# tudocomp/tudocomp

Measured on AMD Instinct MI355X. Metric: input MB/s end-to-end lcpcomp+huffman, higher is better.
Workload: dtype u32

## Files before the change

### tudocomp_amd/csrc/api_compress.hip

```cpp
#include "api.hpp"
#include "bitsink.hpp"

#include <vector>

using namespace tdc;

namespace tdc {

void validate_device_text(Ctx& c, const u8* d_text, size_t n) {
    if (!(c.hist_ptr == d_text && c.hist_n == n)) {
        const size_t mark = c.arena.mark();
        u32* d_hist = c.arena.get<u32>(256);
        HIP_TRY(hipMemsetAsync(d_hist, 0, 256 * sizeof(u32), c.stream));
        text_histogram_add(c, d_text, n, d_hist);
        text_histogram_finish(c, d_text, n, d_hist);
        c.arena.release(mark);
    }
    u8 last = 1;
    HIP_TRY(hipMemcpyAsync(&last, d_text + n - 1, 1, hipMemcpyDeviceToHost, c.stream));
    HIP_TRY(hipStreamSynchronize(c.stream));
    const u32 zeros = c.hist_cache[0];
    if (last != 0) throw ArgError{TDC_GPU_ERR_NO_SENTINEL, "text does not end with a 0 sentinel"};
    if (zeros != 1) throw ArgError{TDC_GPU_ERR_ARG, "text contains 0 bytes besides the sentinel (escape the input first)"};
}

static bool early_is_planned(const Ctx& c, size_t n, u32 threshold, int flatten, int strategy, int enc_coder, const u8* d_text) {
    return strategy == TDC_GPU_COMP_ARRAYS && flatten && enc_coder == 0 && d_text && c.enc_early && c.enc_rec && c.huff_ok &&
           n >= (c.enc_early >= 2 ? (size_t)1 : ((size_t)1 << 20)) && threshold >= 2;
}

void run_textds(Ctx& c, const u8* d_text, size_t n, DevArrays& A, tdc_gpu_stats* st, Events* ev, bool want_phi, const CandWant* cw) {
    A.sa = c.arena.get<u32>(n);
    A.isa = c.arena.get<u32>(n);
    A.phi = nullptr;
    A.plcp = c.arena.get<u32>(n);
    u32* d_max = c.arena.get<u32>(1);
    SAStats ss;
    SAExtra ex;
    ex.lcp8 = c.arena.get<u8>(n + 64);
    const int e0 = ev ? ev->tick() : 0;
    build_suffix_array(c, d_text, n, A.sa, A.isa, &ss, &ex);
    const int e1 = ev ? ev->tick() : 0;
    int e2;
    if (!(ex.mode == 1 && !want_phi && c.phi_lazy)) A.phi = c.arena.get<u32>(n);
    if (ex.mode == 1) {
        CandFused* cf = nullptr;
        if (cw && c.fused_cand && !A.phi && fused_scatter_has_image(c, n)) {
            cf = &A.cand;
            cf->threshold = cw->threshold;
            cf->lcut = factorize_arrays_lcut0(c, n, cw->threshold);
            cf->cls = c.arena.get<u8>(n);
            if (cf->lcut) cf->res8 = c.arena.get<u8>(n);
            if (cw->flen8) cf->flen8 = A.fs.flen8 = c.arena.get<u8>(n + 64); else cf->flen = A.fs.flen = c.arena.get<u32>(n);
            if (c.sel_tile_counts) cf->tilecnt = c.arena.get<u32>(cdiv(n, SEL_TILE_CLASSES));
            cf->acc = c.arena.get<u32>((size_t)CF_COPIES * CF_ACC);
            cf->lvlhist = c.arena.get<u32>(128);
            cf->entries = cf->lvlhist + 64;
        }
        build_isa_phi_plcp_fused(c, A.sa, ex.lcp8, n, A.isa, A.phi, A.plcp, d_max, cf);
        e2 = ev ? ev->tick() : 0;
    } else {
        build_phi(c, A.sa, n, A.phi);
        e2 = ev ? ev->tick() : 0;
        build_plcp(c, d_text, n, A.phi, A.plcp, d_max);
    }
    const int e3 = ev ? ev->tick() : 0;
    A.maxlcp = c.read(d_max);
    if (st) {
        st->maxlcp = A.maxlcp;
        sa_stats(st, ss, &ex);
        if (ev) { ev->span(&st->ms_sa, e0, e1); ev->span(&st->ms_phi, e1, e2); ev->span(&st->ms_plcp, e2, e3); }
    }
}

constexpr size_t FLAT_CHUNK_MIN = (size_t)16 << 20;
constexpr size_t FLAT_CHUNK_MAX = 8;

void run_factorize(Ctx& c, size_t n, DevArrays& A, u32 threshold, int flatten, tdc_gpu_stats* st, Events* ev, int strategy,
                   int enc_coder, const u8* d_text) {
    if (!A.fs.flen) A.fs.flen = c.arena.get<u32>(n);
    A.fs.owner = c.arena.get<u32>(n);
    A.fs.fsrc = c.arena.get<u32>(n);
    A.fs.fpos = c.arena.get<u32>(n);
    A.fs.flenl = threshold >= 2 ? A.fs.fpos + (n + 1) / 2 : nullptr;
    A.fs.cls = c.arena.get<u8>(n + 64);
    const bool early_planned = early_is_planned(c, n, threshold, flatten, strategy, enc_coder, d_text);
    if (early_planned && c.flen_bytes && !A.fs.flen8) A.fs.flen8 = c.arena.get<u8>(n + 64);
    A.fs.want_owner_rem = early_planned ? (u32)c.owner_rem : 0u;
    FactorizeStats fz;
    FlattenStats fl;
    const int e0 = ev ? ev->tick() : 0;
    if (strategy == TDC_GPU_COMP_PLCPPEAKS) plcp_peaks_factorize(c, n, A.phi, A.plcp, threshold, A.fs, &fz.factors);
    else if (strategy == TDC_GPU_COMP_MAXLCP) factorize_max_lcp(c, n, A.isa, A.phi, A.plcp, A.maxlcp, threshold, A.fs, &fz);
    else if (strategy == TDC_GPU_COMP_HEAP) factorize_max_heap(c, n, A.sa, A.isa, A.plcp, A.maxlcp, threshold, A.fs, &fz);
    else factorize_arrays(c, n, A.sa, A.isa, A.phi, A.plcp, A.maxlcp, threshold, A.fs, &fz, A.cand.filled ? &A.cand : nullptr);
    const int e1 = ev ? ev->tick() : 0;
    const bool early = flatten && enc_coder == 0 && d_text && c.enc_early && c.huff_ok && n >= (c.enc_early >= 2 ? (size_t)1 : ((size_t)1 << 20)) &&
                       A.fs.have_list && A.fs.have_cls && A.fs.flenl && A.fs.nfact > 0;
    if (!early) expand_flen8(c, n, A.fs);
    if (early) {
        A.early = encode_early_reserve(c, n, c.enc_rec ? A.fs.nfact : 0);
        u32 K = c.flatten_chunks ? (u32)c.flatten_chunks : (u32)std::min<size_t>(A.fs.nfact / FLAT_CHUNK_MIN, FLAT_CHUNK_MAX);
        K = flatten_chunk_count(K, A.fs.nfact);
        const bool packed = K >= 2 && encode_early_chunks(c, n, A.fs, A.early, K, align_up(encode_bound_coder(n, enc_coder) + 16, 8));
        if (!packed && c.flatten_chunks < 2) K = 1;
        c.wait_for(c.copy_stream, c.stream);
        flatten_factors(c, n, A.fs, &fl, [&](int round) {
            StreamSwap sw(c, c.copy_stream);
            if (round == 1 || round == 2) encode_early_run(c, d_text, n, A.fs, enc_coder, A.early, false);
            else if (round == 0) encode_early_run(c, d_text, n, A.fs, enc_coder, A.early, true);
        }, c.enc_rec ? encode_early_rec(A.early) : nullptr, K,
        packed ? std::function<void(u32, size_t)>([&](u32 k, size_t) { encode_early_chunk_done(c, d_text, n, A.fs, A.early, k); }) : std::function<void(u32, size_t)>());
    } else if (flatten) {
        flatten_factors(c, n, A.fs, &fl);
    } else {
        materialize_sources(c, n, A.fs);
    }
    const int e2 = ev ? ev->tick() : 0;
    if (st) {
        st->factors = fz.factors; st->entries = fz.entries; st->pushes = fz.pushes;
        st->levels = fz.levels; st->mis_rounds = fz.rounds; st->small_levels = fz.small_levels; st->purges = fz.purges; st->window_pass = fz.window_pass; st->window_lcut = fz.window_lcut; st->eager_levels = fz.eager_levels; st->eager_phases = fz.eager_phases;
        st->probes = fz.probes; st->max_push_targets = fz.max_push_targets;
        st->num_flattened = fl.num_flattened; st->max_depth_lb = fl.max_depth_lb; st->flatten_rounds = fl.rounds;
        st->ranges_early = A.early ? encode_early_packed(A.early) : 0u;
        if (ev) { ev->span(&st->ms_factorize, e0, e1); ev->span(&st->ms_flatten, e1, e2); }
    }
}

u8* TextUpload::send(const uint8_t* text, size_t n) {
    if (n < ((size_t)1 << 26)) return upload_plain(c, text, n);
    u8* d_text = c.arena.get<u8>(n + 64);
    u32* d_hist = c.arena.get<u32>(256);
    HIP_TRY(hipMemsetAsync(d_hist, 0, 256 * sizeof(u32), c.stream));
    c.wait_for(c.copy_stream, c.stream);
    const bool try_pre = c.wsort_overlap && c.wpre && wsort_applicable(c, n);
    const size_t CH = try_pre ? (size_t)c.upload_chunks : 8;
    std::vector<size_t> coff;
    {
        std::vector<double> w(CH, 1.0);
        if (try_pre) {
            const size_t T = std::min<size_t>((size_t)c.upload_tail_n, CH - 1);
            double f = 1.0;
            for (size_t k = 0; k < T; ++k) { f *= (double)c.upload_tail_pct / 100.0; w[CH - T + k] = f; }
        }
        double tot = 0; for (double x : w) tot += x;
        coff.push_back(0);
        double acc = 0;
        for (size_t k = 0; k + 1 < CH; ++k) {
            acc += w[k];
            size_t o = ((size_t)((double)n * (acc / tot)) + 4095) & ~(size_t)4095;
            if (o <= coff.back()) o = coff.back() + 4096;
            if (o >= n) break;
            coff.push_back(o);
        }
        coff.push_back(n);
    }
    const size_t nch = coff.size() - 1;
    if (nch > Ctx::CHUNK_EVENTS) throw HipError{hipErrorUnknown, "upload: more chunks than chunk events", (int)__LINE__};
    size_t queued = 0;
    auto queue_copies = [&](size_t upto) {
        for (; queued < nch && queued < upto; ++queued) {
            const size_t off = coff[queued] + (queued ? 64 : 0), end = std::min(coff[queued + 1] + 64, n);
            if (end > off) HIP_TRY(hipMemcpyAsync(d_text + off, text + off, end - off, hipMemcpyHostToDevice, c.copy_stream));
            HIP_TRY(hipEventRecord(c.ev_chunk[queued], c.copy_stream));
// ... 666 lines not shown
```

### tudocomp_amd/csrc/api_ctx.hip

```cpp
#include "api.hpp"
#include "huffman_host.hpp"

#include <strings.h>
#include <ctype.h>

using namespace tdc;

namespace tdc {

int lcpcomp_enc_coder(int coder) {
    const int base = coder & 0xFF, k = coder >> 8;
    if (base == TDC_GPU_CODER_SLE) {
        if (k < 0 || k > 7) throw ArgError{TDC_GPU_ERR_ARG, "sle: kmer must be in 1..7"};
        return 3 | ((k ? k : 3) << 8);
    }
    if (k == 0 && base == TDC_GPU_CODER_HUFF) return 0;
    if (k == 0 && base == TDC_GPU_CODER_ARITH) return 1;
    if (k == 0 && base == TDC_GPU_CODER_ASCII) return 2;
    throw ArgError{TDC_GPU_ERR_UNSUPPORTED, "lcpcomp: coder must be huff, arithmetic, ascii or sle"};
}

void reserve_arena(Ctx& c, size_t bytes) {
    if (c.arena.size < bytes) {
        size_t fr = 0, tot = 0;
// ... 56 lines not shown
    { "phi_lazy",         [](Ctx& c, long v) { c.phi_lazy = v != 0; } },
    { "fs_pair",          [](Ctx& c, long v) { c.fs_pair = v != 0; } },
    { "enc_early",        [](Ctx& c, long v) { c.enc_early = (int)v; } },
    { "owner_rem",        [](Ctx& c, long v) { c.owner_rem = (int)std::min<long>(std::max<long>(v, 0), 8); } },
    { "enc_rec",          [](Ctx& c, long v) { c.enc_rec = v != 0; } },
    { "level_purge",      [](Ctx& c, long v) { c.level_purge = v != 0; } },
    { "level_log",        [](Ctx& c, long v) { c.level_log = v != 0; } },
    { "eager",            [](Ctx& c, long v) { c.eager_levels = v != 0; } },
    { "eager_dump",       [](Ctx& c, long v) { c.eager_dump = v != 0; } },
    { "flen_bytes",       [](Ctx& c, long v) { c.flen_bytes = v != 0; } },
    { "flatten_steps",    [](Ctx& c, long v) { c.flatten_steps = v <= 0 ? (1 << 30) : clampi(v, 1, 1 << 30); } },
    { "flatten_growth",   [](Ctx& c, long v) { c.flatten_growth = clampi(v, 2, 1 << 20); } },
    { "sa_refine",        [](Ctx& c, long v) { c.sa_refine = v != 0; } },
    { "sa_pairs",         [](Ctx& c, long v) { c.sa_pairs = v != 0; } },
    { "sa_stars",         [](Ctx& c, long v) { c.sa_stars = v != 0; } },
    { "sa_fused_init",    [](Ctx& c, long v) { c.sa_fused_init = v != 0; } },
    { "sa_init_syms",     [](Ctx& c, long v) { c.sa_init_syms = clampi(v, 0, 64); } },
    { "radix_lds",        [](Ctx& c, long v) { c.radix_lds = (v >= 0 && v <= 2) ? (int)v : 2; } },
    { "xcd_remap",        [](Ctx& c, long v) { c.xcd_remap = (v >= 0 && v <= 2) ? (int)v : 0; } },
    { "bucket_scatter",   [](Ctx& c, long v) { c.bucket_scatter = v ? 1 : 0; } },
    { "ssort",            [](Ctx& c, long v) { c.ssort = v ? 1 : 0; } },
    { "ssort_levels",     [](Ctx& c, long v) { c.ssort_levels = (v >= 1 && v <= 3) ? (int)v : 0; } },
    { "msd_partition",    [](Ctx& c, long v) { c.msd_partition = v ? 1 : 0; } },
    { "wsort",            [](Ctx& c, long v) { c.wsort = v ? 1 : 0; } },
    { "wsort_min",        [](Ctx& c, long v) { c.wsort_min = v < 4096 ? 4096 : (size_t)v; } },
    { "wsort_syms",       [](Ctx& c, long v) { c.wsort_syms = (v >= 4 && v <= 64) ? (int)v : 0; } },
    { "wsort_kw",         [](Ctx& c, long v) { c.wsort_kw = (v == 1 || v == 2) ? (int)v : 0; } },
    { "wsort_rounds",     [](Ctx& c, long v) { c.wsort_rounds = clampi(v, 0, 100); } },
    { "wsort_smallrun",   [](Ctx& c, long v) { c.wsort_small = v ? 1 : 0; } },
    { "wsort_overlap",    [](Ctx& c, long v) { c.wsort_overlap = v ? 1 : 0; } },
    { "wsort_predig",     [](Ctx& c, long v) { c.wsort_predig = v ? 1 : 0; } },
    { "wsort_prehist",    [](Ctx& c, long v) { c.wsort_prehist = v ? 1 : 0; } },
    { "sa_seg_bigcap",    [](Ctx& c, long v) { c.sa_seg_bigcap = clampi(v, 0, 65536); } },
    { "sa_seg_rounds",    [](Ctx& c, long v) { c.sa_seg_rounds = clampi(v, 0, 2); } },
    { "wsort_run_streams",[](Ctx& c, long v) { c.wsort_run_streams = v != 0; } },
    { "wsort_predig_skip",[](Ctx& c, long v) { c.wsort_predig_skip = clampi(v, 0, 24); } },
    { "wsort_fuse",       [](Ctx& c, long v) { c.wsort_fuse = v ? 1 : 0; } },
    { "wsort_order",      [](Ctx& c, long v) { c.wsort_order = v ? 1 : 0; } },
    { "wsort_two",        [](Ctx& c, long v) { c.wsort_two = (v >= 0 && v <= 2) ? (int)v : 0; } },
    { "wsort_leaf",       [](Ctx& c, long v) { c.wsort_leaf = v == 1024 ? 1024 : 2048; } },
    { "wsort_pack",       [](Ctx& c, long v) { c.wsort_pack = (v == 1024 || v == 4096) ? (int)v : 2048; } },
    { "wsort_cmax",       [](Ctx& c, long v) { c.wsort_cmax = clampi(v, 8, 64); } },
    { "wsort_log",        [](Ctx& c, long v) { c.wsort_log = v != 0; } },
    { "upload_chunks",    [](Ctx& c, long v) { c.upload_chunks = clampi(v, 4, 24); } },
    { "upload_tail_n",    [](Ctx& c, long v) { c.upload_tail_n = clampi(v, 0, 12); } },
    { "upload_tail_pct",  [](Ctx& c, long v) { c.upload_tail_pct = clampi(v, 30, 100); } },
    { "arena_log",        [](Ctx& c, long v) { c.arena_log = v != 0; } },
};
constexpr size_t NOPTIONS = sizeof(OPTIONS) / sizeof(OPTIONS[0]);
const OptionDef FOLD_OPTIONS[] = {
    { "fused_cand",       [](Ctx& c, long v) { c.fused_cand = v != 0; } },
    { "sel_tile_counts",  [](Ctx& c, long v) { c.sel_tile_counts = v != 0; } },
    { "flatten_chunks",   [](Ctx& c, long v) { c.flatten_chunks = clampi(v, 0, (long)FLATTEN_MAX_CHUNKS); } },
    { "repair_recount",   [](Ctx& c, long v) { c.repair_recount = v != 0; } },
    { "repair_table_bits",[](Ctx& c, long v) { c.repair_table_bits = v == 0 ? 0 : clampi(v, 8, 30); } },
    { "repair_log",       [](Ctx& c, long v) { c.repair_log = v != 0; } },
    { "repair_dec_rounds",[](Ctx& c, long v) { c.repair_dec_rounds = clampi(v, 1, 1 << 24); } },
    { "lz_batch_hash_bits",[](Ctx& c, long v) { c.lz_batch_hash_bits = clampi(v, 0, 24); } },
};
constexpr size_t NFOLD = sizeof(FOLD_OPTIONS) / sizeof(FOLD_OPTIONS[0]);
const OptionDef* find_option(const char* name) {
    if (!name) return nullptr;
    if (!strncasecmp(name, "TDC_GPU_", 8)) name += 8;
    for (size_t i = 0; i < NOPTIONS; ++i) if (!strcasecmp(name, OPTIONS[i].name)) return &OPTIONS[i];
    for (size_t i = 0; i < NFOLD; ++i) if (!strcasecmp(name, FOLD_OPTIONS[i].name)) return &FOLD_OPTIONS[i];
    return nullptr;
}
void apply_env_options(tdc_gpu_ctx* ctx) {
    const char* on = getenv("TDC_GPU_DEBUG_KNOBS");
    if (!on || atoi(on) == 0) return;
    for (size_t i = 0; i < NOPTIONS + NFOLD; ++i) {
        const OptionDef& o = i < NOPTIONS ? OPTIONS[i] : FOLD_OPTIONS[i - NOPTIONS];
        char var[64] = "TDC_GPU_";
        size_t k = 8;
        for (const char* q = o.name; *q && k + 1 < sizeof(var); ++q) var[k++] = (char)toupper((unsigned char)*q);
        var[k] = 0;
        if (const char* m = getenv(var)) o.set(ctx->c, atol(m));
    }
}
}

int tdc_gpu_ctx_set_option(tdc_gpu_ctx* ctx, const char* name, long value) {
    if (!ctx) return TDC_GPU_ERR_ARG;
    const OptionDef* o = find_option(name);
    if (!o) return TDC_GPU_ERR_ARG;
    o->set(ctx->c, value);
    return TDC_GPU_OK;
}
int tdc_gpu_option_count(void) { return (int)NOPTIONS; }
const char* tdc_gpu_option_name(int i) { return (i >= 0 && (size_t)i < NOPTIONS) ? OPTIONS[i].name : nullptr; }

int tdc_gpu_ctx_create(int device, tdc_gpu_ctx** out) {
    if (!out) return TDC_GPU_ERR_ARG;
    *out = nullptr;
    int count = 0;
    if (hipGetDeviceCount(&count) != hipSuccess || count <= 0) { (void)hipGetLastError(); return TDC_GPU_ERR_HIP; }
    if (device < 0 || device >= count) return TDC_GPU_ERR_ARG;
    tdc_gpu_ctx* ctx = new (std::nothrow) tdc_gpu_ctx();
    if (!ctx) return TDC_GPU_ERR_OOM;
    ctx->c.huff_ok = huffman_selfcheck();
    ctx->c.device = device;
    ctx->c.wpre = &ctx->pre;
    DeviceGuard dg(device);
    try {
        HIP_TRY(dg.enter());
        HIP_TRY(hipStreamCreateWithFlags(&ctx->c.stream, hipStreamNonBlocking));
// ... 171 lines not shown
```

### tudocomp_amd/csrc/common.hpp

```cpp
#pragma once

#include <hip/hip_runtime.h>
#include <stdint.h>
#include <stddef.h>
#include <stdio.h>
#include <string.h>

namespace tdc {

typedef uint8_t  u8;
typedef uint32_t u32;
typedef uint16_t u16;
typedef uint64_t u64;

constexpr u32 NONE32 = 0xFFFFFFFFu;
constexpr int WAVE = 64;

enum {
    TDC_OK = 0,
    TDC_ERR_HIP = -1,
    TDC_ERR_ARG = -2,
    TDC_ERR_NO_SENTINEL = -3,
    TDC_ERR_TOO_LARGE = -4,
    TDC_ERR_OOM = -5,
// ... 111 lines not shown
    int level_purge = 1;
    int enc_rec = 1;
    int owner_rem = 8;
    int enc_early = 1;
    int fused_cand = 1;
    int sel_tile_counts = 1;
    int fs_pair = 1;
    int small_big = 1;
    int small_pipeline = 1;
    int sa_pairs = 1;
    int sa_stars = 1;
    int sa_refine = 1;
    int sa_fused_init = 1;
    int radix_lds = 1;
    int xcd_remap = 1;
    int window_src = 1;
    int window_lcut = 56;
    int window_halo = 320;
    size_t dec_seg = 0;
    bool phi_lazy = true;
    int dec_lean = 1;
    int dec_parse = 1;
    int window_force_fail = 0;
    int window_large_lists = 0;
    int ssort = 1;
    int ssort_levels = 0;
    int wsort = 1;
    size_t wsort_min = (size_t)1 << 20;
    int wsort_syms = 0;
    int wsort_kw = 0;
    int wsort_rounds = 24;
    int wsort_cmax = 24;
    int wsort_overlap = 1;
    int wsort_prehist = 1;
    bool wsort_count_nonheads = true;
    int sa_seg_bigcap = 65536;
    int sa_seg_rounds = 2;
    int wsort_run_streams = 1;
    int wsort_predig_skip = 4;
    int wsort_predig = 1;
    int wsort_two = 0;
    int wsort_leaf = 2048;
    int wsort_pack = 1024;
    int wsort_order = 1;
    int wsort_fuse = 1;
    int wsort_small = 0;
    int msd_partition = 1;
    int bucket_scatter = 1;
    int upload_tail_n = 3, upload_tail_pct = 60;
    int upload_chunks = 16;
    int flatten_steps = 1;
    int flatten_growth = 8;
    int flatten_chunks = 0;
    int sa_init_syms = 0;
    int dec_done = 1;
    int repair_recount = 0;
    int repair_table_bits = 0;
    int repair_log = 0;
    int repair_dec_rounds = 1024;
    int lz_batch_hash_bits = 0;
    int dec_log = 0, bwt_log = 0, pipe_log = 0, level_log = 0, wsort_log = 0, eager_dump = 0, small_prof = 0, arena_log = 0;

    u32 hist_cache[256] = {};
    const u8* hist_ptr = nullptr;
    size_t hist_n = 0;
    hipStream_t copy_stream = nullptr;
    hipStream_t aux_stream = nullptr;
    hipEvent_t ev_join = nullptr;
    static constexpr size_t CHUNK_EVENTS = 32;
    hipEvent_t ev_chunk[CHUNK_EVENTS] = {};
    hipEvent_t ev_dig2 = nullptr;
    struct WPre* wpre = nullptr;
    u8* d2h_host = nullptr;
    size_t d2h_cap = 0;
    size_t d2h_done = 0;

    bool profiling = false;
    KernelProfile kprof[K_CLASS_COUNT];
    struct Pending { hipEvent_t a, b; int cls; u64 bytes; };
    Pending* pend = nullptr;
    int npend = 0, pend_cap = 0;
    hipEvent_t* ev_pool = nullptr;
    int ev_pool_size = 0, ev_pool_used = 0;

    int prof_begin(int cls, u64 bytes) {
        if (!profiling || npend >= pend_cap || ev_pool_used + 2 > ev_pool_size) return -1;
        Pending& p = pend[npend];
        p.a = ev_pool[ev_pool_used++]; p.b = ev_pool[ev_pool_used++]; p.cls = cls; p.bytes = bytes;
        HIP_TRY(hipEventRecord(p.a, stream));
        return npend++;
    }
    void prof_end(int idx) { if (idx >= 0) HIP_TRY(hipEventRecord(pend[idx].b, stream)); }
    void wait_for(hipStream_t waiter, hipStream_t signaller) {
        HIP_TRY(hipEventRecord(ev_join, signaller));
        HIP_TRY(hipStreamWaitEvent(waiter, ev_join, 0));
    }
    struct ProfScope {
        Ctx& c; int idx;
        ProfScope(Ctx& ctx, int cls, u64 bytes) : c(ctx), idx(ctx.prof_begin(cls, bytes)) {}
        ~ProfScope() { if (idx >= 0) (void)hipEventRecord(c.pend[idx].b, c.stream); }
    };
    void prof_collect() {
        for (int i = 0; i < npend; ++i) {
            float t = 0;
            HIP_TRY(hipEventElapsedTime(&t, pend[i].a, pend[i].b));
            KernelProfile& k = kprof[pend[i].cls];
// ... 274 lines not shown
```

### tudocomp_amd/csrc/encode.hip

```cpp
#include "stages.hpp"
#include "bytestages.hpp"
#include "bitsink.hpp"
#include "prim.hpp"
#include "huffman_host.hpp"
#include "arith.hpp"
#include "decode.hpp"

#include <string.h>
#include <algorithm>
#include <vector>

namespace tdc {

struct CodeTable {
    u64 code[256];
    u8 len[256];
};

struct EncParams {
    u32 W, lbits, dbits, flen_min;
    u32 raw_literals;
    u32 ascii;
    u32 uni;
};
// ... 309 lines not shown
            }
        }
    }
    u64 total;
    const u64 ex = block_exclusive_sum<u64, 4>((u64)sum | ((u64)starts << 40), sm, total);
    const u64 excl = ex & ((1ull << 40) - 1ull);
    if (p0 >= n) return;
    u32 k = REC ? tile_rank[tile] + (u32)(ex >> 40) : 0u;
    BitSink sink;
    sink.out = out;
    sink.pos = base_bits + tile_off[tile] + excl;
    sink.acc = 0;
    sink.cnt = 0;
    u32 prev = prev0;
#pragma unroll
    for (int j = 0; j < ENC_PER_THREAD; ++j) {
        const size_t p = p0 + j;
        if (p < n) {
            const u32 o = cl[j];
            if (o == 0u) {
                if (p == 0 || prev != 0u) {
                    const u32 run = REC ? ((k < z ? rec[k].x : (u32)n) - (u32)p) : fl[j];
                    sink.append(1, 1); sink.append(run, P.dbits);
                }
                if (A.litidx) {
                    const u32 q = A.litidx[p];
                    if (A.amark[q]) sink.append(A.fval[q], 64);
                    if (q == A.lc_index) { sink.append(A.pp_lb, 64); sink.append(~0ull, 64); }
                }
                else if (P.raw_literals) sink.append(ch[j], 8);
                else sink.append(code[ch[j]], clen[ch[j]]);
            } else if (o == 2u) {
                if (p == 0 || prev != 0u) sink.append(0, 1);
                if (REC) {
                    const uint4 r = rec[k++];
                    sink.append(r.w, P.W);
                    sink.append(r.y - P.flen_min, P.lbits);
                } else {
                    sink.append(fsrc[p], P.W);
                    sink.append(fl[j] - P.flen_min, P.lbits);
                }
            }
            prev = o;
        }
    }
    sink.flush();
}

struct PackBounds { u32 end[16]; };
__global__ void pick_u64_kernel(const u64* __restrict__ excl, PackBounds b, u32 parts, u64* __restrict__ out) {
    const u32 q = threadIdx.x;
    if (q < parts) out[q] = (q + 1 < parts) ? excl[b.end[q]] : 0ull;
}
__global__ void range_tiles_kernel(const u32* __restrict__ fpos, u32 z, u32 K, u32* __restrict__ out) {
    const u32 k = threadIdx.x;
    if (k + 1 < K) out[k] = fpos[(u32)((u64)z * (k + 1) / K)] / (u32)ENC_TILE;
}

size_t encode_bound(size_t n) { return 12 * n + 4096; }
size_t encode_bound_coder(size_t n, int coder) { return ((coder & 0xFF) == 2 ? 24 : 12) * n + ((coder & 0xFF) == 3 ? 32768 : 4096); }
size_t encode_bound_uni(size_t n, int coder) { return (coder == 4 ? 8 : coder == 5 ? 9 : 6) * n + 64; }

size_t encode_huff(Ctx& c, const u8* text, size_t n, FactorSpace fs, u8* d_out, size_t out_cap, EncodeStats* st) {
    return encode_stream(c, text, n, fs, 0, d_out, out_cap, st, nullptr);
}

struct EncPrelude { size_t z; u32 hist[256]; EncScalars sc; };
static void encode_prelude_launch(Ctx& c, const u8* text, size_t n, FactorSpace& fs, EncPrelude& pre, u32* r_hist, bool store_runs, u32** o_hist, EncScalars** o_sc) {
    hipStream_t s = c.stream;
    u32* fpos = fs.have_list ? fs.fpos : c.arena.get<u32>(n);
    u32* flist = fs.have_list ? fs.flenl : c.arena.get<u32>(n);
    const size_t z = fs.have_list ? fs.nfact : extract_factors(c, n, fs, fpos, nullptr, flist, n);
    u32* d_hist = r_hist ? r_hist : c.arena.get<u32>(256 + 4);
    EncScalars* d_sc = (EncScalars*)(d_hist + 256);
    EncScalars h_sc = { 0xFFFFFFFFu, 0u, 0u, 0u };
    static_assert(sizeof(EncScalars) == 16, "EncScalars: four words");
    HIP_TRY(hipMemsetAsync(d_sc, 0, sizeof(h_sc), s));
    HIP_TRY(hipMemsetD32Async((hipDeviceptr_t)d_sc, 0xFFFFFFFFu, 1, s));
    HIP_TRY(hipMemsetAsync(d_hist, 0, 256 * sizeof(u32), s));
    if (z) {
        unsigned g = cdiv(z, 256); if (g > 2048) g = 2048;
        Ctx::ProfScope prof(c, K_ENC_GAPS, (u64)z * 12);
        gaps_kernel<<<g, 256, 0, s>>>(fpos, flist, z, n, fs.flen, d_sc, store_runs || !flist);
        LAUNCH_CHECK();
    } else {
        const u32 run = (u32)n;
        HIP_TRY(hipMemcpyAsync(fs.flen, &run, sizeof(u32), hipMemcpyHostToDevice, s));
        h_sc.fdist_max = run;
        HIP_TRY(hipMemcpyAsync(d_sc, &h_sc, sizeof(h_sc), hipMemcpyHostToDevice, s));
    }
    {
        unsigned g = cdiv(n, 256 * 16); if (g > 2048) g = 2048; if (g == 0) g = 1;
        Ctx::ProfScope prof(c, K_ENC_HIST, (u64)n * 5);
        if (fs.have_cls) literal_hist_cls_kernel<<<g, 256, 0, s>>>(text, fs.cls, n, d_hist);
        else literal_hist_kernel<<<g, 256, 0, s>>>(text, plain_owner(fs), n, d_hist);
        LAUNCH_CHECK();
    }
    pre.z = z;
    *o_hist = d_hist; *o_sc = d_sc;
}
static void encode_prelude(Ctx& c, const u8* text, size_t n, FactorSpace& fs, EncPrelude& pre) {
    u32* d_hist; EncScalars* d_sc;
    encode_prelude_launch(c, text, n, fs, pre, nullptr, true, &d_hist, &d_sc);
    u32 h[260];
    c.read_n(d_hist, h, 260);
    memcpy(pre.hist, h, sizeof(pre.hist));
    memcpy(&pre.sc, h + 256, sizeof(pre.sc));
}

// ... 163 lines not shown
EncodeEarly* encode_early_reserve(Ctx& c, size_t n, size_t z_rec) {
    EncodeEarly* E = new EncodeEarly();
    try { encode_reserve(c, n, *E, z_rec); } catch (...) { delete E; throw; }
    return E;
}
void* encode_early_rec(EncodeEarly* E) { return E->rec; }
void encode_early_run(Ctx& c, const u8* text, size_t n, FactorSpace fs, int coder, EncodeEarly* E, bool finish) { encode_first_half(c, text, n, fs, coder, *E, finish); }
void encode_early_free(EncodeEarly* E) { delete E; }

static void pack_begin(Ctx& c, hipStream_t ps, EncodeEarly& E, u8* d_out) {
    if (E.begun) return;
    const HostBitWriter& hw = E.hw;
    HIP_TRY(hipMemsetAsync(d_out, 0, bit_stream_padded(E.out_len), ps));
    if (c.pinned_hdr && hw.bytes.size() <= Ctx::PINNED_HDR) {
        memcpy(c.pinned_hdr, hw.bytes.data(), hw.bytes.size());
        HIP_TRY(hipMemcpyAsync(d_out, c.pinned_hdr, hw.bytes.size(), hipMemcpyHostToDevice, ps));
    } else HIP_TRY(hipMemcpyAsync(d_out, hw.bytes.data(), hw.bytes.size(), hipMemcpyHostToDevice, ps));
    E.begun = true;
}
static void pack_upto(Ctx& c, hipStream_t ps, hipStream_t cs, const u8* text, size_t n, const FactorSpace& fs, EncodeEarly& E, u8* d_out, u32 upto) {
    if (upto <= E.q_done) return;
    const EncParams& P = E.P;
    const ArithDev& A = E.A;
    const CodeTable& tab = E.tab;
    const u64 base_bits = E.base_bits;
    const u64* tile_bits = E.tile_bits;
    const u32 t0 = E.q_done ? E.end.end[E.q_done - 1] : 0u, t1 = upto == E.nb ? E.tiles : E.end.end[upto - 1];
    if (t1 > t0) {
        if (P.uni == (u32)ENC_GAMMA) pack_kernel<ENC_GAMMA><<<t1 - t0, 256, 0, ps>>>(text, plain_owner(fs), fs.flen, fs.fsrc, n, tab, P, A, tile_bits, base_bits, (u64*)d_out, t0);
        else if (P.uni == (u32)ENC_DELTA) pack_kernel<ENC_DELTA><<<t1 - t0, 256, 0, ps>>>(text, plain_owner(fs), fs.flen, fs.fsrc, n, tab, P, A, tile_bits, base_bits, (u64*)d_out, t0);
        else if (P.ascii) pack_kernel<ENC_ASCII><<<t1 - t0, 256, 0, ps>>>(text, plain_owner(fs), fs.flen, fs.fsrc, n, tab, P, A, tile_bits, base_bits, (u64*)d_out, t0);
        else if (fs.have_cls && E.rec) pack_cls_kernel<true><<<t1 - t0, 256, 0, ps>>>(text, fs.cls, fs.flen, fs.fsrc, n, tab, P, A, tile_bits, base_bits, (u64*)d_out, t0, E.rec, E.tile_rank, (u32)E.z_rec);
        else if (fs.have_cls) pack_cls_kernel<false><<<t1 - t0, 256, 0, ps>>>(text, fs.cls, fs.flen, fs.fsrc, n, tab, P, A, tile_bits, base_bits, (u64*)d_out, t0, nullptr, nullptr, 0u);
        else         pack_kernel<ENC_TAB><<<t1 - t0, 256, 0, ps>>>(text, plain_owner(fs), fs.flen, fs.fsrc, n, tab, P, A, tile_bits, base_bits, (u64*)d_out, t0);
        LAUNCH_CHECK();
    }
    E.q_done = upto;
    if (E.overlap && upto < E.nb) {
        const size_t safe = (size_t)((base_bits + E.h_end[upto - 1]) / 64) * 8;
        bool room = true;
        if (E.by_rank && E.ncopy >= PACK_AHEAD) room = hipEventQuery(c.ev_chunk[PACK_CH + E.ncopy - PACK_AHEAD]) == hipSuccess;
        if (safe > E.copied && room) {
            c.wait_for(cs, ps);
            HIP_TRY(hipMemcpyAsync(c.d2h_host + E.copied, d_out + E.copied, safe - E.copied, hipMemcpyDeviceToHost, cs));
            if (E.by_rank) {
                HIP_TRY(hipEventRecord(c.ev_chunk[PACK_CH + E.ncopy++], cs));
                (void)hipStreamQuery(cs);
            }
            E.copied = safe;
        }
    }
}

bool encode_early_chunks(Ctx& c, size_t n, const FactorSpace& fs, EncodeEarly* e, u32 K, size_t out_cap) {
    EncodeEarly& E = *e;
    const size_t z = fs.nfact;
    if (K < 2 || K > FLATTEN_MAX_CHUNKS || K > z || !fs.have_list || !E.rec || E.z_rec != z || E.step != 0 || !c.aux_stream || !c.pinned_hdr || !may_overlap(c, E)) return false;
    E.d_out = c.arena.get<u8>(out_cap);
    E.out_cap = out_cap;
    u32 h[FLATTEN_MAX_CHUNKS] = { 0 };
    const size_t mark = c.arena.mark();
    u32* d_b = c.arena.get<u32>(FLATTEN_MAX_CHUNKS);
    range_tiles_kernel<<<1, 64, 0, c.stream>>>(fs.fpos, (u32)z, K, d_b);
    LAUNCH_CHECK();
    c.read_n(d_b, h, K - 1);
    c.arena.release(mark);
    for (u32 k = 0; k + 1 < K; ++k) E.end.end[k] = std::min<u32>(h[k], E.tiles);
    for (u32 k = K - 1; k < PACK_CH; ++k) E.end.end[k] = E.tiles;
    E.nb = K;
    E.by_rank = true;
    return true;
}
u8* encode_early_out(EncodeEarly* e, size_t* out_cap) { if (e->d_out && out_cap) *out_cap = e->out_cap; return e->d_out; }
u32 encode_early_packed(const EncodeEarly* e) { return e->by_rank ? e->q_done : 0u; }

void encode_early_chunk_done(Ctx& c, const u8* text, size_t n, const FactorSpace& fs, EncodeEarly* e, u32 k) {
    EncodeEarly& E = *e;
    if (!E.by_rank || k >= E.nb) return;
    HIP_TRY(hipEventRecord(c.ev_chunk[k], c.stream));
    E.q_ready = k + 1;
    if (E.step == 2 && E.seq_b && c.publish_test(E.seq_b, 2)) encode_step_c(c, E);
    if (!E.done || bit_stream_padded(E.out_len) > E.out_cap) return;
    if (E.q_ready == E.nb) return;
    const hipStream_t ps = c.copy_stream, cs = c.aux_stream;
    pack_begin(c, ps, E, E.d_out);
    HIP_TRY(hipStreamWaitEvent(ps, c.ev_chunk[k], 0));
    for (u32 q = E.q_done + 1; q <= E.q_ready; ++q) pack_upto(c, ps, cs, text, n, fs, E, E.d_out, q);
    (void)hipStreamQuery(ps);
}

size_t encode_stream(Ctx& c, const u8* text, size_t n, FactorSpace fs, int coder, u8* d_out, size_t out_cap, EncodeStats* st, EncodeEarly* early) {
    EncodeStats local;
    if (!st) st = &local;
    *st = EncodeStats();
    if ((coder & 0xFF) == 3) return encode_sle(c, text, n, fs, (u32)(coder >> 8), d_out, out_cap, st);
    hipStream_t s = c.stream;
    const size_t mark = c.arena.mark();

    EncodeEarly mine;
    if (early && !early->done)
        throw HipError{hipErrorUnknown, "encode: the first half started inside the flatten stage did not complete", (int)__LINE__};
    if (!early) {
        early = &mine;
        encode_reserve(c, n, mine);
        encode_first_half(c, text, n, fs, coder, mine);
    }
    EncodeEarly& E = *early;
    const size_t z = E.z;
    const EncScalars h_sc = E.sc;
    const u64 total_bits = E.total_bits;
    const size_t out_len = E.out_len;
    const size_t padded = bit_stream_padded(out_len);
    if (padded > out_cap) throw HipError{hipErrorOutOfMemory, "encode: output buffer too small", (int)__LINE__};

    if (E.by_rank && d_out != E.d_out) throw HipError{hipErrorUnknown, "encode: the pack behind the flatten ranges writes the buffer reserved for it", (int)__LINE__};
    const hipStream_t ps = E.by_rank ? c.copy_stream : s, cs = E.by_rank ? c.aux_stream : c.copy_stream;
// ... 586 lines not shown
```

### tudocomp_amd/csrc/flatten.hip

```cpp
#include "stages.hpp"
#include "prim.hpp"

#include <stdlib.h>

namespace tdc {

__global__ void fstart_flag_kernel(const u32* __restrict__ flen, const u32* __restrict__ owner, size_t n, u32* __restrict__ flag) {
    const size_t p = (size_t)blockIdx.x * blockDim.x + threadIdx.x;
    if (p >= n) return;
    const u32 o = owner[p];
    flag[p] = (flen[p] != 0 && o != NONE32 && (p == 0 || owner[p - 1] != o)) ? 1u : 0u;
}
__global__ void fstart_scatter_kernel(const u32* __restrict__ flen, const u32* __restrict__ owner, const u32* __restrict__ fsrc,
                                      const u32* __restrict__ offs, size_t n, size_t cap, u32* __restrict__ pos,
                                      u32* __restrict__ src, u32* __restrict__ len) {
    const size_t p = (size_t)blockIdx.x * blockDim.x + threadIdx.x;
    if (p >= n) return;
    const u32 l = flen[p];
    const u32 ow = owner[p];
    if (l != 0 && ow != NONE32 && (p == 0 || owner[p - 1] != ow)) {
        const u32 o = offs[p];
        if (o < cap) {
            pos[o] = (u32)p;
            if (src) src[o] = fsrc[p];
// ... 364 lines not shown
#endif
                    continue; }
            } else {
                ssrc = sr[r].z;
            }
            src[r] = ssrc + d;
            ++dep[r];
        }
    }
#ifdef TDC_FL_PROF
    { const u32 a = wave_reduce_sum(psteps), b = wave_reduce_sum(pwaits);
      if (lane_id() == 0) { atomicAdd(&sc->steps, (unsigned long long)a); atomicAdd(&sc->waits, (unsigned long long)b); } }
#endif
    u32 nflat = 0, mxdep = 0;
#pragma unroll
    for (int r = 0; r < FL_K; ++r) {
        if (fin & (1u << r)) {
            ((u32*)&rec[fi[r]])[3] = src[r];
            if (dep[r]) { ++nflat; mxdep = max(mxdep, dep[r]); }
        }
    }
    const u32 wmask = valid & ~fin;
    u32 total;
    u32 off = block_exclusive_sum<u32, 4>((u32)__popc(wmask), sm, total);
    if (threadIdx.x == 0) s_base = total ? atomicAdd(&sc->waiting, total) : 0u;
    __syncthreads();
    off += s_base;
#pragma unroll
    for (int r = 0; r < FL_K; ++r)
        if (wmask & (1u << r)) next[off++] = make_uint4(fi[r], len[r], src[r], dep[r]);
    nflat = wave_reduce_sum(nflat);
    mxdep = wave_reduce_max(mxdep);
    if (lane_id() == 0 && nflat) { atomicAdd(&sc->num_flattened, nflat); atomicMax(&sc->max_depth, mxdep); }
}

__global__ void flatten_commit_kernel(size_t z, const uint4* __restrict__ rec, u32* __restrict__ fsrc) {
    const size_t i = (size_t)blockIdx.x * blockDim.x + threadIdx.x;
    if (i >= z) return;
    const uint4 q = rec[i];
    if (q.w != q.z) fsrc[q.x] = q.w;
}

void materialize_sources(Ctx& c, size_t n, FactorSpace& fs) {
    if (!fs.src_prio) return;
    if (n) {
        if (fs.have_list) { if (fs.nfact) sources_fill_kernel<<<cdiv(fs.nfact, 256), 256, 0, c.stream>>>(fs.fpos, fs.nfact, fs.src_prio, fs.src_sa, fs.src_n, fs.fsrc); }
        else sources_fill_pos_kernel<<<cdiv(n, 256), 256, 0, c.stream>>>(fs.flen, n, fs.src_prio, fs.src_sa, fs.src_n, fs.fsrc);
        LAUNCH_CHECK();
    }
    fs.src_prio = nullptr;
}

void flatten_factors(Ctx& c, size_t n, FactorSpace fs, FlattenStats* st, const std::function<void(int)>& between, void* rec_keep,
                     u32 chunks, const std::function<void(u32, size_t)>& chunk_done) {
    if (fs.src_prio && !rec_keep) materialize_sources(c, n, fs);
    FlattenStats local;
    if (!st) st = &local;
    *st = FlattenStats();
    if (n == 0) { if (between) between(0); return; }
    hipStream_t s = c.stream;
    const size_t mark = c.arena.mark();
    u32* fpos = fs.have_list ? fs.fpos : c.arena.get<u32>(n);
    const size_t z = fs.have_list ? fs.nfact : extract_factors(c, n, fs, fpos, nullptr, nullptr, n);
    if (z == 0) { if (between) between(0); c.arena.release(mark); return; }
    const u32 K = flatten_chunk_count(chunks ? chunks : (u32)c.flatten_chunks, z);
    uint4* rec = rec_keep ? (uint4*)rec_keep : (uint4*)c.arena.alloc(z * sizeof(uint4));
    FlattenScalars* d_sc = (FlattenScalars*)c.arena.alloc(sizeof(FlattenScalars));
    HIP_TRY(hipMemsetAsync(d_sc, 0, sizeof(FlattenScalars), s));
    const unsigned gz = cdiv(z, 256);
    flatten_init_kernel<<<gz, 256, 0, s>>>(fpos, z, fs.flen, fs.fsrc, rec, fs.have_list ? fs.flenl : nullptr, fs.src_prio, fs.src_sa, fs.src_n);
    LAUNCH_CHECK();
    const size_t cmax = (z + K - 1) / K;
    uint4* work[2] = { (uint4*)c.arena.alloc(cmax * sizeof(uint4)), nullptr };
    u32 flat_growth = (u32)c.flatten_growth;
    if (flat_growth < 2) flat_growth = 2;
    for (u32 k = 0; k < K; ++k) {
        const size_t r0 = flatten_chunk_start(z, k, K), r1 = flatten_chunk_start(z, k + 1, K);
        u32 waiting = (u32)(r1 - r0);
        int cur_w = -1;
        u32 max_steps = (u32)c.flatten_steps;
        if (max_steps == 0) max_steps = 1u << 30;
        u32 stalled = 0;
        while (waiting) {
            const int nxt = cur_w < 0 ? 0 : (cur_w ^ 1);
            if (!work[nxt]) work[nxt] = (uint4*)c.arena.alloc((K == 1 ? (size_t)waiting : cmax) * sizeof(uint4));
            HIP_TRY(hipMemsetAsync(&d_sc->waiting, 0, sizeof(u32), s));
            {
                Ctx::ProfScope prof(c, K_FLATTEN_ROUND, (u64)waiting * 52);
                const u32 rb = fs.owner_rem_bits;
                const unsigned g = cdiv(waiting, 256 * FL_K);
                if (cur_w < 0) { if (rb) flatten_round_kernel<true, true><<<g, 256, 0, s>>>(nullptr, waiting, n, fs.owner, rec, work[nxt], d_sc, max_steps, rb, (u32)r0);
                                 else flatten_round_kernel<true, false><<<g, 256, 0, s>>>(nullptr, waiting, n, fs.owner, rec, work[nxt], d_sc, max_steps, 0u, (u32)r0); }
                else { if (rb) flatten_round_kernel<false, true><<<g, 256, 0, s>>>(work[cur_w], waiting, n, fs.owner, rec, work[nxt], d_sc, max_steps, rb, 0u);
                       else flatten_round_kernel<false, false><<<g, 256, 0, s>>>(work[cur_w], waiting, n, fs.owner, rec, work[nxt], d_sc, max_steps, 0u, 0u); }
                LAUNCH_CHECK();
            }
            if (between) between((int)st->rounds + 1);
            const u32 now = c.read(&d_sc->waiting);
            st->rounds++;
            if (c.level_log) {
                const FlattenScalars hs = c.read(d_sc);
                fprintf(stderr, "flatten round %u (range %u of %u): %u waiting -> %u (budget %u steps; cumulative: %llu visits, %llu of them waits)\n", st->rounds, k + 1, K, waiting, now, max_steps, hs.steps, hs.waits);
            }
            stalled = (now == waiting) ? stalled + 1 : 0;
            if (now > waiting || (now == waiting && max_steps >= (1u << 30)) || stalled > 40)
                throw HipError{hipErrorUnknown, "flatten: rounds made no progress", (int)__LINE__};
            waiting = now;
            cur_w = nxt;
            if (max_steps < (1u << 30)) max_steps = (max_steps > (1u << 30) / flat_growth) ? (1u << 30) : max_steps * flat_growth;
        }
        if (chunk_done) chunk_done(k, r1);
    }
    if (between) between(0);
    if (!rec_keep) {
        flatten_commit_kernel<<<gz, 256, 0, s>>>(z, rec, fs.fsrc);
        LAUNCH_CHECK();
    }
    FlattenScalars h = c.read(d_sc);
    st->num_flattened = h.num_flattened;
    st->max_depth_lb = h.max_depth;
    c.arena.release(mark);
}

}
```

### tudocomp_amd/csrc/stages.hpp

```cpp
#pragma once
#include "common.hpp"
#include <functional>

namespace tdc {

size_t escape_device(Ctx& c, const u8* d_in, size_t n, u8* d_out);
size_t count_escapes_device(Ctx& c, const u8* d_in, size_t n);

struct SAStats { u32 rounds = 0; u32 sym_bits = 0; u32 init_syms = 0; u64 sorted_elems = 0;
                 u32 wide_kw = 0;  u32 text_rounds = 0; u64 wide_nonheads = 0;
                 u32 overlapped = 0;
                 u64 pair_resolved = 0;
                 u64 star_chains = 0;  };
struct SAExtra { u8* lcp8 = nullptr; int mode = 0; };

void build_suffix_array(Ctx& c, const u8* text, size_t n, u32* sa, u32* isa, SAStats* st, SAExtra* ex = nullptr);
struct CandFused {
    u32 threshold = 0, lcut = 0;
    u8* cls = nullptr;
    u8* res8 = nullptr;
    u8* flen8 = nullptr;
    u32* flen = nullptr;
    u32* tilecnt = nullptr;
    u32* acc = nullptr;
// ... 8 lines not shown
void text_histogram_add(Ctx& c, const u8* part, size_t len, u32* d_hist);
void text_histogram_finish(Ctx& c, const u8* text, size_t n, const u32* d_hist);

void build_phi(Ctx& c, const u32* sa, size_t n, u32* phi);
void build_plcp(Ctx& c, const u8* text, size_t n, const u32* phi, u32* plcp, u32* d_maxlcp);
void build_lce_with_carry(Ctx& c, const u8* text, size_t n, const u32* src, u32* len, u32* d_max);
void build_lcp(Ctx& c, const u32* sa, const u32* plcp, size_t n, u32* lcp);

struct FactorSpace {
    u32* flen = nullptr;
    u8* flen8 = nullptr;
    u32* owner = nullptr;
    u32* fsrc = nullptr;
    u32* fpos = nullptr;
    u32* flenl = nullptr;
    size_t nfact = 0;
    bool have_list = false;
    u8* cls = nullptr;
    bool have_cls = false;
    u32 want_owner_rem = 0;
    u32 owner_rem_bits = 0;
    const u32* src_prio = nullptr;
    const u32* src_sa = nullptr;
    size_t src_n = 0;
};
inline const u32* plain_owner(const FactorSpace& fs) {
    if (fs.owner_rem_bits) throw HipError{hipErrorUnknown, "owner[] carries remainder bits (FactorSpace::owner_rem_bits): this stage reads plain ranks", (int)__LINE__};
    return fs.owner;
}
void materialize_sources(Ctx& c, size_t n, FactorSpace& fs);

struct FactorizeStats { u64 factors = 0; u32 maxlcp = 0; u32 levels = 0; u32 rounds = 0; u64 pushes = 0; u64 entries = 0; u32 small_levels = 0; u32 purges = 0;
                        u32 window_pass = 0;
                        u32 window_lcut = 0;
                        u32 probes = 0;
                        u32 max_push_targets = 0;
                        u32 eager_levels = 0, eager_phases = 0;  };

void factorize_arrays(Ctx& c, size_t n, const u32* sa, u32* isa, const u32* phi, u32* plcp, u32 maxlcp,
                      u32 threshold, FactorSpace& fs, FactorizeStats* st, const CandFused* cf = nullptr);

void build_owner(Ctx& c, size_t n, FactorSpace& fs);
void expand_flen8(Ctx& c, size_t n, FactorSpace& fs);

void plcp_peaks_factorize(Ctx& c, size_t n, const u32* phi, const u32* plcp, u32 threshold, FactorSpace& fs, u64* nfactors);
void factorize_max_lcp(Ctx& c, size_t n, u32* isa, const u32* phi, u32* plcp, u32 maxlcp, u32 threshold, FactorSpace& fs,
                       FactorizeStats* st);

void factorize_max_heap(Ctx& c, size_t n, const u32* sa, const u32* isa, const u32* plcp, u32 maxlcp, u32 threshold, FactorSpace& fs,
                        FactorizeStats* st);

struct FlattenStats { u64 num_flattened = 0; u64 max_depth_lb = 0; u32 rounds = 0; };
constexpr u32 FLATTEN_MAX_CHUNKS = 16;
inline u32 flatten_chunk_count(u32 want, size_t z) { return (u32)std::max<size_t>(1, std::min<size_t>(std::min<size_t>(want, FLATTEN_MAX_CHUNKS), z)); }
inline size_t flatten_chunk_start(size_t z, u32 k, u32 K) { return (size_t)((u64)z * k / K); }
void flatten_factors(Ctx& c, size_t n, FactorSpace fs, FlattenStats* st, const std::function<void(int)>& between = {}, void* rec_keep = nullptr,
                     u32 chunks = 0, const std::function<void(u32, size_t)>& chunk_done = {});

size_t extract_factors(Ctx& c, size_t n, FactorSpace fs, u32* pos, u32* src, u32* len, size_t cap);
void scatter_factors(Ctx& c, size_t n, const u32* pos, const u32* src, const u32* len, size_t z, FactorSpace fs);

struct EncodeStats { u64 factors = 0; u64 flen_min = 0, flen_max = 0, fdist_max = 0; u64 out_bits = 0; u32 sigma = 0; };
size_t encode_huff(Ctx& c, const u8* text, size_t n, FactorSpace fs, u8* d_out, size_t out_cap, EncodeStats* st);
struct EncodeEarly;
size_t encode_stream(Ctx& c, const u8* text, size_t n, FactorSpace fs, int coder, u8* d_out, size_t out_cap, EncodeStats* st, EncodeEarly* early = nullptr);
EncodeEarly* encode_early_reserve(Ctx& c, size_t n, size_t z_rec = 0);
void* encode_early_rec(EncodeEarly* e);
void encode_early_run(Ctx& c, const u8* text, size_t n, FactorSpace fs, int coder, EncodeEarly* e, bool finish = true);
void encode_early_free(EncodeEarly* e);
bool encode_early_chunks(Ctx& c, size_t n, const FactorSpace& fs, EncodeEarly* e, u32 K, size_t out_cap);
void encode_early_chunk_done(Ctx& c, const u8* text, size_t n, const FactorSpace& fs, EncodeEarly* e, u32 k);
u8* encode_early_out(EncodeEarly* e, size_t* out_cap);
u32 encode_early_packed(const EncodeEarly* e);

size_t encode_bound(size_t n);
size_t encode_bound_coder(size_t n, int coder);
size_t encode_bound_uni(size_t n, int coder);

struct LzssStats { u64 factors = 0; };
void lzss_lcp_factorize(Ctx& c, const u8* text, size_t n, const u32* sa, const u32* isa, u32 threshold, FactorSpace fs,
                        LzssStats* st);

}
#include <vector>
namespace tdc {
struct DecodeStats { u64 factors = 0; u32 rounds = 0; u32 device_parse = 0; };
struct StreamFormatError { const char* what; };
struct Sink {
    u8* into = nullptr; size_t cap = 0;
    u8* owned = nullptr;
    uint8_t** out = nullptr; size_t* out_len = nullptr;
    bool keep = false;
    Sink() = default;
    Sink(Sink&& o) : into(o.into), cap(o.cap), owned(o.owned), out(o.out), out_len(o.out_len), keep(o.keep) { o.owned = nullptr; }
    Sink(const Sink&) = delete;
    Sink& operator=(const Sink&) = delete;
    ~Sink() { free(owned); }
    u8* release() { u8* r = owned; owned = nullptr; return r; }
};
size_t decode_lzss(Ctx& c, const u8* stream, size_t len, int coder, Sink& out, DecodeStats* st);
bool decode_lzss_uni(Ctx& c, const u8* stream, size_t len, int kind, Sink& out, DecodeStats* st, size_t* n_out);
struct DecodeTooLarge { u64 n; };
size_t decode_lz78_gamma(Ctx& c, const u8* stream, size_t len, Sink& out, size_t* need, DecodeStats* st);
size_t lz78_parse_host(const u8* in, size_t n, std::vector<u32>& ids, std::vector<u8>& chars, bool* leftover_is_high);
size_t lz78_gamma_encode(Ctx& c, const u32* d_ids, const u8* d_chars, size_t z, u8* d_out, size_t out_cap);
size_t gamma_encode_items(Ctx& c, const u32* d_ids, const u8* d_chars, size_t z, u8* d_out, size_t out_cap);

size_t lzw_parse_host(const u8* in, size_t n, std::vector<u32>& codes);
size_t lzw_encode(Ctx& c, const u32* d_codes, size_t z, bool bit, u8* d_out, size_t out_cap);
constexpr size_t LZW_DEVICE_MIN = (size_t)64 << 10;
size_t decode_lzw(Ctx& c, const u8* stream, size_t len, bool bit, Sink& out, size_t* need, DecodeStats* st);

constexpr u32 LZSS_SW_MAX_WINDOW = 4096;
size_t lzss_sw_tokens(Ctx& c, const u8* d_text, size_t n, u32 window, u32 threshold, u32** tokpos, u32** fac);
size_t lzss_sw_factor_list(Ctx& c, const u32* tokpos, const u32* fac, size_t ntok, u32* d_pos, u32* d_src, u32* d_len);
struct LzssSwStats { u64 factors = 0; u32 flen_max = 0; bool truncates = false; };
size_t lzss_sw_encode_tokens(Ctx& c, const u8* d_text, const u32* tokpos, const u32* fac, size_t ntok, u32 window, int kind,
                             u8* d_out, size_t out_cap, LzssSwStats* st);
size_t lzss_sw_bound(size_t n, u32 window, int kind);
bool decode_lzss_sw(Ctx& c, const u8* stream, size_t len, int kind, u32 window, Sink& out, size_t* need, DecodeStats* st, size_t* n_out);
int lzss_sw_decode_host(const u8* in, size_t len, int coder, u32 window, std::vector<u8>& text);

struct LzssSwBatch {
// ... 52 lines not shown
```

Baseline: 8791.

## Split flatten into a large first chunk followed by halving tail chunks

Replaces the equal-size flatten chunking (up to 8 chunks of at least 16M factors) with explicit rank ranges. By default the first chunk takes 37% of the factors and each later chunk halves the remainder until the tail drops to 8M, and the chunked path is only used at 32M factors or more. The aim is to start the overlapped early encoding of completed chunks sooner and to keep the final, unoverlapped chunk small. It also adds options for custom range shapes and generalizes the range-tile kernel. The cost is more chunks and more per-chunk launch and sync overhead, plus a larger first work buffer.

```diff
diff --git a/tudocomp_amd/csrc/api_compress.hip b/tudocomp_amd/csrc/api_compress.hip
--- a/tudocomp_amd/csrc/api_compress.hip
+++ b/tudocomp_amd/csrc/api_compress.hip
@@ -73,8 +73,16 @@
     }
 }
 
-constexpr size_t FLAT_CHUNK_MIN = (size_t)16 << 20;
-constexpr size_t FLAT_CHUNK_MAX = 8;
+constexpr size_t FLAT_AUTO_MIN = (size_t)32 << 20;
+constexpr u32 FLAT_FIRST_PCT = 37;
+constexpr size_t FLAT_TAIL = (size_t)8 << 20;
+
+static FlattenRanges choose_flatten_ranges(const Ctx& c, size_t z) {
+    if (c.flatten_chunks) return flatten_ranges_equal(z, (u32)c.flatten_chunks);
+    if (c.flatten_shape) return flatten_ranges_weighted(z, c.flatten_shape);
+    if (!c.flatten_tail && z < FLAT_AUTO_MIN) return flatten_ranges_equal(z, 1);
+    return flatten_ranges_shaped(z, c.flatten_first ? (size_t)c.flatten_first : (size_t)((u64)z * FLAT_FIRST_PCT / 100), c.flatten_tail ? (size_t)c.flatten_tail : FLAT_TAIL);
+}
 
 void run_factorize(Ctx& c, size_t n, DevArrays& A, u32 threshold, int flatten, tdc_gpu_stats* st, Events* ev, int strategy,
                    int enc_coder, const u8* d_text) {
@@ -100,16 +108,15 @@
     if (!early) expand_flen8(c, n, A.fs);
     if (early) {
         A.early = encode_early_reserve(c, n, c.enc_rec ? A.fs.nfact : 0);
-        u32 K = c.flatten_chunks ? (u32)c.flatten_chunks : (u32)std::min<size_t>(A.fs.nfact / FLAT_CHUNK_MIN, FLAT_CHUNK_MAX);
-        K = flatten_chunk_count(K, A.fs.nfact);
-        const bool packed = K >= 2 && encode_early_chunks(c, n, A.fs, A.early, K, align_up(encode_bound_coder(n, enc_coder) + 16, 8));
-        if (!packed && c.flatten_chunks < 2) K = 1;
+        FlattenRanges R = choose_flatten_ranges(c, A.fs.nfact);
+        const bool packed = R.K >= 2 && encode_early_chunks(c, n, A.fs, A.early, R, align_up(encode_bound_coder(n, enc_coder) + 16, 8));
+        if (!packed && c.flatten_chunks < 2) R = flatten_ranges_equal(A.fs.nfact, 1);
         c.wait_for(c.copy_stream, c.stream);
         flatten_factors(c, n, A.fs, &fl, [&](int round) {
             StreamSwap sw(c, c.copy_stream);
             if (round == 1 || round == 2) encode_early_run(c, d_text, n, A.fs, enc_coder, A.early, false);
             else if (round == 0) encode_early_run(c, d_text, n, A.fs, enc_coder, A.early, true);
-        }, c.enc_rec ? encode_early_rec(A.early) : nullptr, K,
+        }, c.enc_rec ? encode_early_rec(A.early) : nullptr, &R,
         packed ? std::function<void(u32, size_t)>([&](u32 k, size_t) { encode_early_chunk_done(c, d_text, n, A.fs, A.early, k); }) : std::function<void(u32, size_t)>());
     } else if (flatten) {
         flatten_factors(c, n, A.fs, &fl);
diff --git a/tudocomp_amd/csrc/api_ctx.hip b/tudocomp_amd/csrc/api_ctx.hip
--- a/tudocomp_amd/csrc/api_ctx.hip
+++ b/tudocomp_amd/csrc/api_ctx.hip
@@ -132,6 +132,9 @@
     { "fused_cand",       [](Ctx& c, long v) { c.fused_cand = v != 0; } },
     { "sel_tile_counts",  [](Ctx& c, long v) { c.sel_tile_counts = v != 0; } },
     { "flatten_chunks",   [](Ctx& c, long v) { c.flatten_chunks = clampi(v, 0, (long)FLATTEN_MAX_CHUNKS); } },
+    { "flatten_shape",    [](Ctx& c, long v) { c.flatten_shape = (u64)v; } },
+    { "flatten_first",    [](Ctx& c, long v) { c.flatten_first = v < 0 ? 0 : v; } },
+    { "flatten_tail",     [](Ctx& c, long v) { c.flatten_tail = v < 0 ? 0 : v; } },
     { "repair_recount",   [](Ctx& c, long v) { c.repair_recount = v != 0; } },
     { "repair_table_bits",[](Ctx& c, long v) { c.repair_table_bits = v == 0 ? 0 : clampi(v, 8, 30); } },
     { "repair_log",       [](Ctx& c, long v) { c.repair_log = v != 0; } },
diff --git a/tudocomp_amd/csrc/common.hpp b/tudocomp_amd/csrc/common.hpp
--- a/tudocomp_amd/csrc/common.hpp
+++ b/tudocomp_amd/csrc/common.hpp
@@ -187,6 +187,9 @@
     int flatten_steps = 1;
     int flatten_growth = 8;
     int flatten_chunks = 0;
+    u64 flatten_shape = 0;
+    long flatten_first = 0;
+    long flatten_tail = 0;
     int sa_init_syms = 0;
     int dec_done = 1;
     int repair_recount = 0;
diff --git a/tudocomp_amd/csrc/encode.hip b/tudocomp_amd/csrc/encode.hip
--- a/tudocomp_amd/csrc/encode.hip
+++ b/tudocomp_amd/csrc/encode.hip
@@ -385,9 +385,9 @@
     const u32 q = threadIdx.x;
     if (q < parts) out[q] = (q + 1 < parts) ? excl[b.end[q]] : 0ull;
 }
-__global__ void range_tiles_kernel(const u32* __restrict__ fpos, u32 z, u32 K, u32* __restrict__ out) {
+__global__ void range_tiles_kernel(const u32* __restrict__ fpos, FlattenRanges R, u32* __restrict__ out) {
     const u32 k = threadIdx.x;
-    if (k + 1 < K) out[k] = fpos[(u32)((u64)z * (k + 1) / K)] / (u32)ENC_TILE;
+    if (k + 1 < R.K) out[k] = fpos[R.start[k + 1]] / (u32)ENC_TILE;
 }
 
 size_t encode_bound(size_t n) { return 12 * n + 4096; }
@@ -657,16 +657,19 @@
     }
 }
 
-bool encode_early_chunks(Ctx& c, size_t n, const FactorSpace& fs, EncodeEarly* e, u32 K, size_t out_cap) {
+bool encode_early_chunks(Ctx& c, size_t n, const FactorSpace& fs, EncodeEarly* e, const FlattenRanges& R, size_t out_cap) {
     EncodeEarly& E = *e;
     const size_t z = fs.nfact;
-    if (K < 2 || K > FLATTEN_MAX_CHUNKS || K > z || !fs.have_list || !E.rec || E.z_rec != z || E.step != 0 || !c.aux_stream || !c.pinned_hdr || !may_overlap(c, E)) return false;
+    const u32 K = R.K;
+    bool ranges_ok = K >= 2 && K <= FLATTEN_MAX_CHUNKS && R.start[0] == 0 && R.start[K] == z;
+    for (u32 k = 0; ranges_ok && k < K; ++k) ranges_ok = R.start[k] < R.start[k + 1];
+    if (!ranges_ok || !fs.have_list || !E.rec || E.z_rec != z || E.step != 0 || !c.aux_stream || !c.pinned_hdr || !may_overlap(c, E)) return false;
     E.d_out = c.arena.get<u8>(out_cap);
     E.out_cap = out_cap;
     u32 h[FLATTEN_MAX_CHUNKS] = { 0 };
     const size_t mark = c.arena.mark();
     u32* d_b = c.arena.get<u32>(FLATTEN_MAX_CHUNKS);
-    range_tiles_kernel<<<1, 64, 0, c.stream>>>(fs.fpos, (u32)z, K, d_b);
+    range_tiles_kernel<<<1, 64, 0, c.stream>>>(fs.fpos, R, d_b);
     LAUNCH_CHECK();
     c.read_n(d_b, h, K - 1);
     c.arena.release(mark);
diff --git a/tudocomp_amd/csrc/flatten.hip b/tudocomp_amd/csrc/flatten.hip
--- a/tudocomp_amd/csrc/flatten.hip
+++ b/tudocomp_amd/csrc/flatten.hip
@@ -440,7 +440,7 @@
 }
 
 void flatten_factors(Ctx& c, size_t n, FactorSpace fs, FlattenStats* st, const std::function<void(int)>& between, void* rec_keep,
-                     u32 chunks, const std::function<void(u32, size_t)>& chunk_done) {
+                     const FlattenRanges* ranges, const std::function<void(u32, size_t)>& chunk_done) {
     if (fs.src_prio && !rec_keep) materialize_sources(c, n, fs);
     FlattenStats local;
     if (!st) st = &local;
@@ -451,19 +451,21 @@
     u32* fpos = fs.have_list ? fs.fpos : c.arena.get<u32>(n);
     const size_t z = fs.have_list ? fs.nfact : extract_factors(c, n, fs, fpos, nullptr, nullptr, n);
     if (z == 0) { if (between) between(0); c.arena.release(mark); return; }
-    const u32 K = flatten_chunk_count(chunks ? chunks : (u32)c.flatten_chunks, z);
+    const FlattenRanges R = ranges ? *ranges : flatten_ranges_equal(z, (u32)c.flatten_chunks);
+    if (R.start[0] != 0 || R.start[R.K] != z) throw HipError{hipErrorUnknown, "flatten: the rank ranges do not cover the factor list", (int)__LINE__};
+    const u32 K = R.K;
     uint4* rec = rec_keep ? (uint4*)rec_keep : (uint4*)c.arena.alloc(z * sizeof(uint4));
     FlattenScalars* d_sc = (FlattenScalars*)c.arena.alloc(sizeof(FlattenScalars));
     HIP_TRY(hipMemsetAsync(d_sc, 0, sizeof(FlattenScalars), s));
     const unsigned gz = cdiv(z, 256);
     flatten_init_kernel<<<gz, 256, 0, s>>>(fpos, z, fs.flen, fs.fsrc, rec, fs.have_list ? fs.flenl : nullptr, fs.src_prio, fs.src_sa, fs.src_n);
     LAUNCH_CHECK();
-    const size_t cmax = (z + K - 1) / K;
+    const size_t cmax = R.largest();
     uint4* work[2] = { (uint4*)c.arena.alloc(cmax * sizeof(uint4)), nullptr };
     u32 flat_growth = (u32)c.flatten_growth;
     if (flat_growth < 2) flat_growth = 2;
     for (u32 k = 0; k < K; ++k) {
-        const size_t r0 = flatten_chunk_start(z, k, K), r1 = flatten_chunk_start(z, k + 1, K);
+        const size_t r0 = R.start[k], r1 = R.start[k + 1];
         u32 waiting = (u32)(r1 - r0);
         int cur_w = -1;
         u32 max_steps = (u32)c.flatten_steps;
diff --git a/tudocomp_amd/csrc/stages.hpp b/tudocomp_amd/csrc/stages.hpp
--- a/tudocomp_amd/csrc/stages.hpp
+++ b/tudocomp_amd/csrc/stages.hpp
@@ -84,10 +84,50 @@
 
 struct FlattenStats { u64 num_flattened = 0; u64 max_depth_lb = 0; u32 rounds = 0; };
 constexpr u32 FLATTEN_MAX_CHUNKS = 16;
-inline u32 flatten_chunk_count(u32 want, size_t z) { return (u32)std::max<size_t>(1, std::min<size_t>(std::min<size_t>(want, FLATTEN_MAX_CHUNKS), z)); }
-inline size_t flatten_chunk_start(size_t z, u32 k, u32 K) { return (size_t)((u64)z * k / K); }
+struct FlattenRanges {
+    u32 K = 1;
+    size_t start[FLATTEN_MAX_CHUNKS + 1] = { 0 };
+    size_t largest() const { size_t m = 0; for (u32 k = 0; k < K; ++k) m = std::max(m, start[k + 1] - start[k]); return m; }
+};
+inline FlattenRanges flatten_ranges_of_sizes(size_t z, const size_t* size, size_t count) {
+    FlattenRanges r;
+    size_t at = 0;
+    for (size_t i = 0; i < count && r.K < FLATTEN_MAX_CHUNKS; ++i) {
+        at = size[i] < z - at ? at + size[i] : z;
+        if (at >= z) break;
+        if (at > r.start[r.K - 1]) r.start[r.K++] = at;
+    }
+    r.start[r.K] = z;
+    return r;
+}
+inline FlattenRanges flatten_ranges_equal(size_t z, u32 want) {
+    FlattenRanges r;
+    r.K = (u32)std::max<size_t>(1, std::min<size_t>(std::min<size_t>(want, FLATTEN_MAX_CHUNKS), z));
+    for (u32 k = 0; k <= r.K; ++k) r.start[k] = (size_t)((u64)z * k / r.K);
+    return r;
+}
+inline FlattenRanges flatten_ranges_weighted(size_t z, u64 shape) {
+    u32 w[16], nw = 0;
+    u64 total = 0;
+    for (int s = 60; s >= 0; s -= 4) { const u32 x = (u32)(shape >> s) & 15u; if (nw || x) { w[nw++] = x; total += x; } }
+    size_t size[16], at = 0;
+    u64 acc = 0;
+    for (u32 i = 0; i < nw; ++i) {
+        acc += w[i];
+        const size_t b = (size_t)((u64)z * acc / total);
+        size[i] = b - at; at = b;
+    }
+    return flatten_ranges_of_sizes(z, size, nw);
+}
+inline FlattenRanges flatten_ranges_shaped(size_t z, size_t first, size_t tail) {
+    size_t size[FLATTEN_MAX_CHUNKS], count = 0;
+    size_t left = z - std::min(first, z);
+    size[count++] = first;
+    while (count + 1 < FLATTEN_MAX_CHUNKS && left > std::max<size_t>(tail, 1)) { size[count] = left / 2; left -= size[count++]; }
+    return flatten_ranges_of_sizes(z, size, count);
+}
 void flatten_factors(Ctx& c, size_t n, FactorSpace fs, FlattenStats* st, const std::function<void(int)>& between = {}, void* rec_keep = nullptr,
-                     u32 chunks = 0, const std::function<void(u32, size_t)>& chunk_done = {});
+                     const FlattenRanges* ranges = nullptr, const std::function<void(u32, size_t)>& chunk_done = {});
 
 size_t extract_factors(Ctx& c, size_t n, FactorSpace fs, u32* pos, u32* src, u32* len, size_t cap);
 void scatter_factors(Ctx& c, size_t n, const u32* pos, const u32* src, const u32* len, size_t z, FactorSpace fs);
@@ -100,7 +140,7 @@
 void* encode_early_rec(EncodeEarly* e);
 void encode_early_run(Ctx& c, const u8* text, size_t n, FactorSpace fs, int coder, EncodeEarly* e, bool finish = true);
 void encode_early_free(EncodeEarly* e);
-bool encode_early_chunks(Ctx& c, size_t n, const FactorSpace& fs, EncodeEarly* e, u32 K, size_t out_cap);
+bool encode_early_chunks(Ctx& c, size_t n, const FactorSpace& fs, EncodeEarly* e, const FlattenRanges& R, size_t out_cap);
 void encode_early_chunk_done(Ctx& c, const u8* text, size_t n, const FactorSpace& fs, EncodeEarly* e, u32 k);
 u8* encode_early_out(EncodeEarly* e, size_t* out_cap);
 u32 encode_early_packed(const EncodeEarly* e);
```

After: 8413. -4.3%, worse.
